# PH8411/image-matching

Measured on AMD Instinct MI355X. Metric: image-pairs/sec (640x480, 1024 kpts, 30 Sinkhorn iters), higher is better.
Workload: dtype f32

## Files before the change

### image-matching_amd/csrc/conv1ab_wino24h.hip

```cpp
#include "imx_kernels.h"
#include "wino24_pk.h"
#include <cstdio>
#include <cstdlib>
#include <type_traits>

namespace imx {

typedef float f32x4 __attribute__((ext_vector_type(4)));
typedef float f32x2 __attribute__((ext_vector_type(2)));
typedef _Float16 f16x8 __attribute__((ext_vector_type(8)));
typedef _Float16 f16x2 __attribute__((ext_vector_type(2)));
typedef unsigned u32x4v __attribute__((ext_vector_type(4)));

namespace {
constexpr int OH = 8, OW = 16;
constexpr int RH = OH + 2, RW = OW + 2;
constexpr int IMG_H = RH + 2, IMG_W = RW + 2;
constexpr int RSH = 34;
constexpr int RAWSZ = 192 * RSH;
constexpr int NPOS = 24;
constexpr int VPLANE = NPOS * 4 * 16 * 8;
constexpr int UPOS = 2 * 4 * 64 * 8;
constexpr int RING = 6;

// ... 8 lines not shown
  h[0] = (_Float16)x[0]; h[1] = (_Float16)x[1];
  const float r0 = __builtin_amdgcn_fdot2(h, lo, x[0], false);
  const float r1 = __builtin_amdgcn_fdot2(h, hi, x[1], false);
  m[0] = (_Float16)r0; m[1] = (_Float16)r1;
}
__device__ __forceinline__ float v_scale_of_bound(float bound) {
  unsigned e = (__builtin_bit_cast(unsigned, bound) >> 23) & 0xffu;
  e = e < 60u ? 60u : e > 200u ? 200u : e;
  return __builtin_bit_cast(float, (261u - e) << 23);
}

__global__ __launch_bounds__(256, 2) void conv1ab_wino24h(ConvArgs p, int tiles_x, int tiles_y, int ntiles) {
  extern __shared__ __attribute__((aligned(16))) unsigned char smem_1h[];
  _Float16* Vp = reinterpret_cast<_Float16*>(smem_1h);
  float* raw = reinterpret_cast<float*>(smem_1h + 2 * VPLANE * 2);
  float* img = raw + RAWSZ;
  float* wmax = img + IMG_H * IMG_W;

  const int tid = threadIdx.x, lane = tid & 63, wave = tid >> 6;
  const int cb = wave;
  const int H = p.H, W = p.W, Cout = p.Cout;
  const __amdgpu_buffer_rsrc_t ur = __builtin_amdgcn_make_buffer_rsrc((void*)p.wuh, 0, 2 * NPOS * UPOS * 2, 0x00020000);
  const int uoff_lane = (cb * 64 + lane) * 16;

  const int n = lane & 15, kq = lane >> 4;
  const float c2 = kq == 0 ? 1.f : 0.f, a2 = kq == 1 ? 1.f : 0.f;
  float wa[4][3];
  int toff[3];
#pragma unroll
  for (int ks = 0; ks < 3; ++ks) {
    const int tap = 4 * ks + kq;
    toff[ks] = tap < 9 ? (tap / 3) * IMG_W + tap % 3 : 0;
#pragma unroll
    for (int cbk = 0; cbk < 4; ++cbk) {
      const float* src = tap < 9 ? p.w1 + tap * 64 + cbk * 16 + n : p.b1 + cbk * 16 + n;
      const float v = *(tap <= 9 ? src : p.b1);
      wa[cbk][ks] = tap <= 9 ? v : 0.f;
    }
  }
  const int tk = lane & 3, tw = lane >> 2, twr = tw >> 2, twc = tw & 3;
  const int ra = wave == 0 ? 0 : wave == 2 ? 2 : 1, rb = wave == 0 ? 2 : wave == 1 ? 2 : wave == 2 ? 1 : 3;
  const float sg = wave == 1 ? 1.f : -1.f;
  const f32x2 sg2 = {sg, sg};
  const f32x2 m5 = {-5.f, -5.f};
  const float* rpa = raw + ((2 * twr + ra) * RW + 4 * twc) * RSH + 2 * tk;
  const float* rpb = raw + ((2 * twr + rb) * RW + 4 * twc) * RSH + 2 * tk;
  _Float16* vwr = Vp + (wave * 4 * 16 + tw) * 8 + 2 * tk;
  const _Float16* vrd = Vp + lane * 8;

  const int per = (ntiles + (int)gridDim.x - 1) / (int)gridDim.x;
  const int t_begin = (int)blockIdx.x * per, t_end = t_begin + per < ntiles ? t_begin + per : ntiles;
  int tx = t_begin % tiles_x, ty = (t_begin / tiles_x) % tiles_y, b = t_begin / (tiles_x * tiles_y);
  const int ipy = tid / IMG_W - 2, ipx = tid % IMG_W - 2;
  auto fetch_px = [&](int ftx, int fty, int fb, bool live) -> float {
// ... 24 lines not shown
  };
  const f32x4 bs4 = *reinterpret_cast<const f32x4*>(p.bias + cb * 16 + 4 * (lane >> 4));
  u32x4v ub[RING][2];
  auto u_load = [&](int slot, int chv, int pos) __attribute__((always_inline)) {
    const int so = __builtin_amdgcn_readfirstlane((chv * NPOS + pos) * (UPOS * 2));
    ub[slot][0] = __builtin_amdgcn_raw_buffer_load_b128(ur, uoff_lane, so, 0);
    ub[slot][1] = __builtin_amdgcn_raw_buffer_load_b128(ur, uoff_lane, so + 4 * 64 * 16, 0);
  };
#pragma unroll
  for (int g = 0; g < RING; ++g) u_load(g, 0, g);
  __builtin_amdgcn_s_waitcnt(0x0F70);

  f32x4 acc[NPOS];
  const f32x2 k8 = {8.f, 8.f};
  const f32x4 zero4c = {0.f, 0.f, 0.f, 0.f};
  float sv = 1.f;

  auto conv1a_half = [&](int half, int x0, int y0) __attribute__((always_inline)) {
    const f32x4 zero4 = {0.f, 0.f, 0.f, 0.f};
#pragma unroll
    for (int j = 0; j < 3; ++j) {
      const int pp = (3 * wave + j) * 16 + n;
      const int py = gpy[j], px = gpx[j];
      const int gy = y0 + py - 1, gx = x0 + px - 1;
      const float m = (pp < RH * RW && gy >= 0 && gy < H && gx >= 0 && gx < W) ? sv : 0.f;
      const float* ip = img + py * IMG_W + px;
      float bv[3];
      bv[0] = ip[toff[0]] * m;
      bv[1] = ip[toff[1]] * m;
      bv[2] = (ip[toff[2]] * c2 + a2) * m;
#pragma unroll
      for (int cl = 0; cl < 2; ++cl) {
        f32x4 d = zero4;
#pragma unroll
        for (int ks = 0; ks < 3; ++ks) d = __builtin_amdgcn_mfma_f32_16x16x4f32(half ? wa[2 + cl][ks] : wa[cl][ks], bv[ks], d, 0, 0, 0);
        typedef int i32x4 __attribute__((ext_vector_type(4)));
        d = __builtin_bit_cast(f32x4, __builtin_elementwise_max(__builtin_bit_cast(i32x4, d), (i32x4){0, 0, 0, 0}));
        float* o = raw + pp * RSH + cl * 16 + 4 * kq;
        *reinterpret_cast<f32x2*>(o) = (f32x2){d[0], d[1]};
        *reinterpret_cast<f32x2*>(o + 2) = (f32x2){d[2], d[3]};
      }
    }
  };
  auto transform = [&]() __attribute__((always_inline)) {
#pragma unroll
    for (int q = 0; q < 4; ++q) {
      f32x2 o[6], T[6];
#pragma unroll
      for (int bb = 0; bb < 6; ++bb)
        o[bb] = pk_fma(sg2, *reinterpret_cast<const f32x2*>(rpb + 8 * q + bb * RSH), *reinterpret_cast<const f32x2*>(rpa + 8 * q + bb * RSH));
      const W24Half hb = w24_batch_a(o, m5);
      w24_batch_b(o, hb, T);
#pragma unroll
      for (int jj = 0; jj < 6; ++jj) {
        f16x2 h, m;
        split_h2(T[jj], h, m);
        _Float16* d = vwr + ((jj * 4 * 4 + q) * 16) * 8;
// ... 18 lines not shown
      acc[pp + 1] = __builtin_amdgcn_mfma_f32_16x16x32_f16(ah1, bm[1], FIRST ? zero4c : acc[pp + 1], 0, 0, 0);
      acc[pp] = __builtin_amdgcn_mfma_f32_16x16x32_f16(am0, bh[0], acc[pp], 0, 0, 0);
      acc[pp + 1] = __builtin_amdgcn_mfma_f32_16x16x32_f16(am1, bh[1], acc[pp + 1], 0, 0, 0);
      acc[pp] = __builtin_amdgcn_mfma_f32_16x16x32_f16(ah0, bh[0], acc[pp], 0, 0, 0);
      acc[pp + 1] = __builtin_amdgcn_mfma_f32_16x16x32_f16(ah1, bh[1], acc[pp + 1], 0, 0, 0);
#pragma unroll
      for (int e = 0; e < 2; ++e) {
        const int np = pp + e + RING;
        if (np < NPOS) u_load((pp + e) % RING, c, np);
        else u_load((pp + e) % RING, c ^ 1, np - NPOS);
      }
      __builtin_amdgcn_sched_barrier(0);
    }
  };

  for (int t = t_begin; t < t_end; ++t) {
    const int x0 = tx * OW, y0 = ty * OH, bcur = b;
    if (tid < IMG_H * IMG_W) img[tid] = pre;
    {
      float mx = fabsf(pre);
#pragma unroll
      for (int o = 32; o >= 1; o >>= 1) mx = fmaxf(mx, __shfl_xor(mx, o));
      if (lane == 0) wmax[wave] = mx;
    }
    if (++tx == tiles_x) { tx = 0; if (++ty == tiles_y) { ty = 0; ++b; } }
    pre = fetch_px(tx, ty, b, t + 1 < t_end);
    __syncthreads();
    {
      const float imax = fmaxf(fmaxf(wmax[0], wmax[1]), fmaxf(wmax[2], wmax[3]));
      sv = __builtin_bit_cast(float, __builtin_amdgcn_readfirstlane(__builtin_bit_cast(int, v_scale_of_bound(fmaf(imax, p.c1a_l1, p.c1a_bmax)))));
    }
    conv1a_half(0, x0, y0);
    __syncthreads();
    transform();
    __syncthreads();
    mfma_phase(BoolC<true>{}, 0);
    conv1a_half(1, x0, y0);
    __syncthreads();
    transform();
    __syncthreads();
    mfma_phase(BoolC<false>{}, 1);

    {
      const float inv = p.u_scale_inv / sv;
      const f32x4 inv4 = {inv, inv, inv, inv};
      f32x4 y[2][4];
      w24_output_transform(acc, k8, y);
      const f32x4 zero4 = {0.f, 0.f, 0.f, 0.f};
      const int wr = (lane & 15) >> 2, wc = lane & 3;
      const int Ho = H >> 1, Wo = W >> 1;
      const __amdgpu_buffer_rsrc_t ors = __builtin_amdgcn_make_buffer_rsrc((void*)(p.out + (size_t)bcur * Ho * Wo * Cout), 0, Ho * Wo * Cout * 4, 0x00020000);
      const bool outb = p.out_blocked != 0;
// ... 8 lines not shown
        const int ox = (x0 >> 1) + 2 * wc + hh;
        const unsigned off = (oy < Ho && ox < Wo) ? (unsigned)((oy * Wo + ox) * opx + choff) : 0x7ffffff0u;
        __builtin_amdgcn_raw_buffer_store_b128(__builtin_bit_cast(u32x4, v), ors, (int)off, 0, 0);
        if (p.amax_out) {
          if (bcur != am_b) { am_flush(); am_b = bcur; }
          am_run = max(am_run, __builtin_bit_cast(unsigned, fmaxf(fmaxf(v[0], v[1]), fmaxf(v[2], v[3]))));
        }
      }
    }
  }
  if (p.amax_out) am_flush();
}
}

bool conv1ab_wino24h_supported(const ConvArgs& a) {
  return a.first && a.pool && a.Cin == 64 && a.Cout == 64 && a.wuh && a.u_scale_inv > 0.f && a.c1a_l1 > 0.f;
}

hipError_t launch_conv1ab_wino24h(const ConvArgs& a, hipStream_t s) {
  if (!conv1ab_wino24h_supported(a)) return hipErrorInvalidValue;
  const int tiles_x = (a.W + OW - 1) / OW, tiles_y = (a.H + OH - 1) / OH, ntiles = tiles_x * tiles_y * a.B;
  const size_t lds = (size_t)2 * VPLANE * 2 + (size_t)(RAWSZ + IMG_H * IMG_W + 4) * sizeof(float);
  static int ncu = 0;
  if (!ncu) {
    int dev = 0;
    hipDeviceProp_t prop;
    if (hipGetDevice(&dev) != hipSuccess || hipGetDeviceProperties(&prop, dev) != hipSuccess) return hipErrorUnknown;
    ncu = prop.multiProcessorCount;
  }
  static unsigned long long attr = 0;
  raise_lds_limit(reinterpret_cast<const void*>(conv1ab_wino24h), (int)lds, attr);
  const dim3 grid((unsigned)(ntiles < 2 * ncu ? ntiles : 2 * ncu));
  last_form = "conv1ab_wino24h:f16x2";
  hipLaunchKernelGGL(conv1ab_wino24h, grid, dim3(256), lds, s, a, tiles_x, tiles_y, ntiles);
  return hipGetLastError();
}

// ... 2 lines not shown
```

### image-matching_amd/csrc/conv1ab_wino24p.hip

```cpp
#include "imx_kernels.h"
#include "wino24_pk.h"
#include <cstdint>
#include <cstdio>
#include <cstdlib>
#include <type_traits>

namespace imx {

typedef float f32x4 __attribute__((ext_vector_type(4)));
typedef float f32x2 __attribute__((ext_vector_type(2)));
typedef _Float16 f16x8 __attribute__((ext_vector_type(8)));
typedef _Float16 f16x2 __attribute__((ext_vector_type(2)));
typedef unsigned u32x4v __attribute__((ext_vector_type(4)));

namespace {
constexpr int OH = 8, OW = 16;
constexpr int RH = OH + 2, RW = OW + 2;
constexpr int IMG_H = RH + 2, IMG_W = RW + 2;
constexpr int IMG_N = IMG_H * IMG_W;
constexpr int RSH = 34;
constexpr int RAWSZ = 192 * RSH;
constexpr int NPOS = 24, NLP = 12, NG = 2;
constexpr int VPLANE = NPOS * 4 * 16 * 8;
constexpr int VGRP = 2 * VPLANE;
// ... 17 lines not shown
}
__device__ __forceinline__ int lane_now() {
  int l;
  asm volatile("v_mbcnt_lo_u32_b32 %0, -1, 0\n\tv_mbcnt_hi_u32_b32 %0, -1, %0" : "=v"(l));
  return l;
}
__device__ __forceinline__ float v_scale_of_bound(float bound) {
  unsigned e = (__builtin_bit_cast(unsigned, bound) >> 23) & 0xffu;
  e = e < 60u ? 60u : e > 200u ? 200u : e;
  return __builtin_bit_cast(float, (261u - e) << 23);
}

__global__ __launch_bounds__(512) void conv1ab_wino24p(ConvArgs p, int tiles_x, int tiles_y, int ntiles) {
  extern __shared__ __attribute__((aligned(16))) unsigned char smem_1p[];
  float* raw = reinterpret_cast<float*>(smem_1p + NG * VGRP * 2);
  float* img = raw + NG * RAWSZ;
  float* wmax = img + NG * IMG_N;
  unsigned* amax_tab = reinterpret_cast<unsigned*>(wmax + 8);
  const unsigned lds0 = (unsigned)(uintptr_t)(__attribute__((address_space(3))) unsigned char*)smem_1p;

  const int tid = threadIdx.x, lane = tid & 63;
  const int wave_s = __builtin_amdgcn_readfirstlane(tid >> 6);
  const int cb = wave_s & 3, ph = wave_s >> 2;
  const int tq = wave_s & 3, tg = wave_s >> 2;
  const int H = p.H, W = p.W, Cout = p.Cout;
  const __amdgpu_buffer_rsrc_t ur = __builtin_amdgcn_make_buffer_rsrc((void*)p.wuh, 0, 2 * NPOS * UPOS * 2, 0x00020000);
  const int uoff_lane = (cb * 64 + lane) * 16 + ph * NLP * (UPOS * 2);
  typedef const float __attribute__((address_space(4)))* cf32p;
  const cf32p bias_c = (cf32p)(uintptr_t)p.bias;

  const int n = lane & 15, kq = lane >> 4;
  const float c2 = kq == 0 ? 1.f : 0.f, a2 = kq == 1 ? 1.f : 0.f;
  float wa[4][3];
  int toff[3];
#pragma unroll
  for (int ks = 0; ks < 3; ++ks) {
    const int tap = 4 * ks + kq;
    toff[ks] = tap < 9 ? (tap / 3) * IMG_W + tap % 3 : 0;
#pragma unroll
    for (int cbk = 0; cbk < 4; ++cbk) {
      const float* src = tap < 9 ? p.w1 + tap * 64 + cbk * 16 + n : p.b1 + cbk * 16 + n;
      const float v = *(tap <= 9 ? src : p.b1);
      wa[cbk][ks] = tap <= 9 ? v : 0.f;
    }
  }
  const int tk = lane & 3, tw = lane >> 2, twr = tw >> 2, twc = tw & 3;
  const f32x2 m5 = {-5.f, -5.f}, one2 = {1.f, 1.f}, mone2 = {-1.f, -1.f};
  const float* rp = raw + tg * RAWSZ + ((2 * twr) * RW + 4 * twc) * RSH + 8 * tq + 2 * tk;
  _Float16* const vwr = (_Float16*)((__attribute__((address_space(3))) unsigned char*)(uintptr_t)(lds0 + (unsigned)(tg * (VGRP * 2) + tq * 256 + lane * 4)));
  const _Float16 *vrdK, *vrdS;
  {
    unsigned a = lds0 + (unsigned)(ph * (VGRP * 2) + ph * NLP * 1024 + lane * 16);
    unsigned b = lds0 + (unsigned)((1 - ph) * (VGRP * 2) + ph * NLP * 1024 + lane * 16);
    asm volatile("" : "+v"(a), "+v"(b));
    vrdK = (const _Float16*)((__attribute__((address_space(3))) unsigned char*)(uintptr_t)a);
    vrdS = (const _Float16*)((__attribute__((address_space(3))) unsigned char*)(uintptr_t)b);
  }

  const int npairs = (ntiles + NG - 1) / NG;
  const int per = (npairs + (int)gridDim.x - 1) / (int)gridDim.x;
// ... 34 lines not shown
  }
  u32x4v ub[RING][2];
  auto u_load = [&](int slot, int chv, int lp) __attribute__((always_inline)) {
    const int pos = lp;
    const int so = __builtin_amdgcn_readfirstlane((chv * NPOS + pos) * (UPOS * 2));
    ub[slot][0] = __builtin_amdgcn_raw_buffer_load_b128(ur, uoff_lane, so, 0);
    ub[slot][1] = __builtin_amdgcn_raw_buffer_load_b128(ur, uoff_lane, so + 4 * 64 * 16, 0);
  };
  for (int i = tid; i < AMAX_SLOTS; i += 512) amax_tab[i] = 0;
#pragma unroll
  for (int g = 0; g < RING; ++g) u_load(g, 0, g);

  f32x4 accK[NLP], accS[NLP];
  const f32x2 k8 = {8.f, 8.f};
  const f32x4 zero4c = {0.f, 0.f, 0.f, 0.f};
  float sv = 1.f;
  float* const rawt = raw + tg * RAWSZ;
  const float* const imgt = img + tg * IMG_N;

  auto conv1a_block = [&](int half, int j, int x0, int y0, float svb) __attribute__((always_inline)) {
    const f32x4 zero4 = {0.f, 0.f, 0.f, 0.f};
    {
      const int pp = (3 * tq + j) * 16 + n;
      const int py = gpy[j], px = gpx[j];
      const int gy = y0 + py - 1, gx = x0 + px - 1;
      const float m = (pp < RH * RW && gy >= 0 && gy < H && gx >= 0 && gx < W) ? svb : 0.f;
      const float* ip = imgt + py * IMG_W + px;
      float bv[3];
      bv[0] = ip[toff[0]] * m;
      bv[1] = ip[toff[1]] * m;
      bv[2] = (ip[toff[2]] * c2 + a2) * m;
#pragma unroll
      for (int cl = 0; cl < 2; ++cl) {
        f32x4 d = zero4;
#pragma unroll
        for (int ks = 0; ks < 3; ++ks) d = __builtin_amdgcn_mfma_f32_16x16x4f32(half ? wa[2 + cl][ks] : wa[cl][ks], bv[ks], d, 0, 0, 0);
        typedef int i32x4 __attribute__((ext_vector_type(4)));
        d = __builtin_bit_cast(f32x4, __builtin_elementwise_max(__builtin_bit_cast(i32x4, d), (i32x4){0, 0, 0, 0}));
        float* o = rawt + pp * RSH + cl * 16 + 4 * kq;
        *reinterpret_cast<f32x2*>(o) = (f32x2){d[0], d[1]};
        *reinterpret_cast<f32x2*>(o + 2) = (f32x2){d[2], d[3]};
      }
    }
  };
  auto conv1a_half = [&](int half, int x0, int y0, float svb) __attribute__((always_inline)) {
#pragma unroll
    for (int j = 0; j < 3; ++j) conv1a_block(half, j, x0, y0, svb);
  };
  auto v_store2 = [&](int pos, f16x2 h, f16x2 m) __attribute__((always_inline)) {
    *reinterpret_cast<f16x2*>(vwr + pos * 512) = h;
    *reinterpret_cast<f16x2*>(vwr + VPLANE + pos * 512) = m;
  };
  auto transform = [&]() __attribute__((always_inline)) {
    f32x2 r1[6], r2[6], rx[6];
    auto row_load = [&](f32x2 (&d)[6], int row) __attribute__((always_inline)) {
#pragma unroll
      for (int bb = 0; bb < 6; ++bb) d[bb] = *reinterpret_cast<const f32x2*>(rp + (row * RW + bb) * RSH);
    };
    auto row_out = [&](int i, f32x2 sg2, const f32x2 (&bq)[6], const f32x2 (&aq)[6]) __attribute__((always_inline)) {
      f32x2 o[6], T[6];
// ... 5 lines not shown
      for (int jj = 0; jj < 6; ++jj) {
        f16x2 h, m;
        split_h2(T[jj], h, m);
        v_store2(jj * 4 + i, h, m);
      }
    };
    row_load(r1, 1);
    row_load(r2, 2);
    row_load(rx, 0);
    row_out(1, one2, r2, r1);
    row_out(2, mone2, r1, r2);
    row_out(0, mone2, r2, rx);
    row_load(rx, 3);
    row_out(3, mone2, rx, r1);
  };
  auto mfma_phase = [&](auto firstc, int c, int x0, int y0, float svb) __attribute__((always_inline)) {
    constexpr bool FIRST = decltype(firstc)::value;
    f16x8 bq[2][4];
    auto b_load = [&](int buf, int lp) __attribute__((always_inline)) {
      const int po = lp * 512;
      bq[buf][0] = *reinterpret_cast<const f16x8*>(vrdK + po);
      bq[buf][1] = *reinterpret_cast<const f16x8*>(vrdK + VPLANE + po);
      bq[buf][2] = *reinterpret_cast<const f16x8*>(vrdS + po);
      bq[buf][3] = *reinterpret_cast<const f16x8*>(vrdS + VPLANE + po);
    };
    b_load(0, 0);
#pragma unroll
    for (int lp = 0; lp < NLP; ++lp) {
      const int buf = lp & 1;
      if (lp + 1 < NLP) b_load(buf ^ 1, lp + 1);
      __builtin_amdgcn_sched_barrier(0);
// ... 11 lines not shown
        else u_load(lp % RING, c ^ 1, np - NLP);
      }
      __builtin_amdgcn_sched_barrier(0);
      if ((lp & 3) == 1) {
        conv1a_block(FIRST ? 1 : 0, lp >> 2, x0, y0, svb);
        __builtin_amdgcn_sched_barrier(0);
      }
    }
  };

  unsigned amax_run = 0;
  const int Ho = H >> 1, Wo = W >> 1;
  const bool outb = p.out_blocked != 0;
  const int opx = outb ? 32 : Cout * 4;
  __syncthreads();
  auto image_to_lds = [&]() __attribute__((always_inline)) {
    const int ln = lane_now(), t8n = (wave_s & 3) * 64 + ln;
    if (t8n < IMG_N) img[tg * IMG_N + t8n] = pre;
    unsigned mb = __builtin_bit_cast(unsigned, fabsf(pre));
    mb = max(mb, (unsigned)__builtin_amdgcn_update_dpp(0, (int)mb, 0xb1, 0xf, 0xf, true));
    mb = max(mb, (unsigned)__builtin_amdgcn_update_dpp(0, (int)mb, 0x4e, 0xf, 0xf, true));
    mb = max(mb, (unsigned)__builtin_amdgcn_update_dpp(0, (int)mb, 0x141, 0xf, 0xf, true));
    mb = max(mb, (unsigned)__builtin_amdgcn_update_dpp(0, (int)mb, 0x140, 0xf, 0xf, true));
    const unsigned m01 = max((unsigned)__builtin_amdgcn_readlane((int)mb, 0), (unsigned)__builtin_amdgcn_readlane((int)mb, 16));
    const unsigned m23 = max((unsigned)__builtin_amdgcn_readlane((int)mb, 32), (unsigned)__builtin_amdgcn_readlane((int)mb, 48));
    if (ln == 0) wmax[wave_s] = __builtin_bit_cast(float, max(m01, m23));
  };
  auto scale_from_lds = [&]() __attribute__((always_inline)) -> float {
    const float* wm = wmax + 4 * tg;
    const float imax = fmaxf(fmaxf(wm[0], wm[1]), fmaxf(wm[2], wm[3]));
    return __builtin_bit_cast(float, __builtin_amdgcn_readfirstlane(__builtin_bit_cast(int, v_scale_of_bound(fmaf(imax, p.c1a_l1, p.c1a_bmax)))));
  };
  int x0 = tx * OW, y0 = ty * OH, bcur = tlive ? b : 0, lcur = tlive;
  image_to_lds();
  next_tile();
  pre = fetch_px(q_begin + 1 < q_end);
  __syncthreads();
  sv = scale_from_lds();
  conv1a_half(0, x0, y0, sv);
  __syncthreads();
  for (int q = q_begin; q < q_end; ++q) {
    transform();
    __syncthreads();
    mfma_phase(BoolC<true>{}, 0, x0, y0, sv);
    __syncthreads();
    const int x0n = tx * OW, y0n = ty * OH, bn = tlive ? b : 0, ln = tlive;
    image_to_lds();
    next_tile();
    pre = fetch_px(q + 2 < q_end);
    transform();
    __syncthreads();
    const float svn = scale_from_lds();
    mfma_phase(BoolC<false>{}, 1, x0n, y0n, svn);
    __syncthreads();

    typedef __attribute__((address_space(3))) f32x4* lds4p;
    const int lq = lane_now();
    const unsigned xw = lds0 + (unsigned)(wave_s * XCH + lq * 16), xr = lds0 + (unsigned)((wave_s ^ 4) * XCH + lq * 16);
    f32x4 bs4;
    {
      const int bo = __builtin_amdgcn_readfirstlane(cb * 16);
      typedef const f32x4 __attribute__((address_space(4)))* cf4p;
      const cf4p b4 = (cf4p)(bias_c + bo);
      const f32x4 b0 = b4[0], b1 = b4[1], b2 = b4[2], b3 = b4[3];
      const int kq2 = lq >> 4;
#pragma unroll
      for (int qq = 0; qq < 4; ++qq) bs4[qq] = kq2 == 0 ? b0[qq] : kq2 == 1 ? b1[qq] : kq2 == 2 ? b2[qq] : b3[qq];
// ... 17 lines not shown
      gs0[jj] = *(lds4p)(uintptr_t)(xr + (2 * jj) * 1024);
      gs1[jj] = *(lds4p)(uintptr_t)(xr + (2 * jj + 1) * 1024);
    }
    __syncthreads();

    f32x4 y[2][4];
    {
      auto cols = [&](const f32x4 (&a0)[3], const f32x4 (&a1)[3], const f32x4 (&b0)[3], const f32x4 (&b1)[3]) __attribute__((always_inline)) {
        const f32x4 s0[6] = {a0[0], a0[1], a0[2], b0[0], b0[1], b0[2]}, s1[6] = {a1[0], a1[1], a1[2], b1[0], b1[1], b1[2]};
        w24_out_cols(s0, s1, k8, y);
      };
      if (ph == 0) { cols(sK0, sK1, gs0, gs1); asm volatile("" ::: "memory"); }
      else { cols(gs0, gs1, sK0, sK1); asm volatile("; order 1" ::: "memory"); }
    }
    {
      const float inv = p.u_scale_inv / sv;
      const f32x4 inv4 = {inv, inv, inv, inv};
      const f32x4 zero4 = {0.f, 0.f, 0.f, 0.f};
      const int wr = (lq & 15) >> 2, wc = lq & 3;
      const int bu = __builtin_amdgcn_readfirstlane(bcur), lv = __builtin_amdgcn_readfirstlane(lcur);
      const __amdgpu_buffer_rsrc_t ors = __builtin_amdgcn_make_buffer_rsrc((void*)(p.out + (size_t)bu * Ho * Wo * Cout), 0, lv ? Ho * Wo * Cout * 4 : 0, 0x00020000);
      const int choff = outb ? (cb * 2 + (lq >> 5)) * (Ho * Wo * 32) + ((lq >> 4) & 1) * 16 : (cb * 16 + 4 * (lq >> 4)) * 4;
      typedef unsigned u32x4 __attribute__((__vector_size__(4 * sizeof(unsigned))));
      const int oy = (y0 >> 1) + wr;
#pragma unroll
      for (int hh = 0; hh < 2; ++hh) {
        const f32x4 mx4 = __builtin_elementwise_max(__builtin_elementwise_max(y[0][2 * hh], y[0][2 * hh + 1]), __builtin_elementwise_max(y[1][2 * hh], y[1][2 * hh + 1]));
        const f32x4 v = __builtin_elementwise_max(__builtin_elementwise_fma(mx4, inv4, bs4), zero4);
        const int ox = (x0 >> 1) + 2 * wc + hh;
        const unsigned off = (oy < Ho && ox < Wo) ? (unsigned)((oy * Wo + ox) * opx + choff) : 0x7ffffff0u;
        __builtin_amdgcn_raw_buffer_store_b128(__builtin_bit_cast(u32x4, v), ors, (int)off, 0, 0);
        amax_run = max(amax_run, __builtin_bit_cast(unsigned, fmaxf(fmaxf(v[0], v[1]), fmaxf(v[2], v[3]))));
      }
      if (p.amax_out) {
        unsigned mb = amax_run;
        mb = max(mb, (unsigned)__builtin_amdgcn_update_dpp(0, (int)mb, 0xb1, 0xf, 0xf, true));
        mb = max(mb, (unsigned)__builtin_amdgcn_update_dpp(0, (int)mb, 0x4e, 0xf, 0xf, true));
        mb = max(mb, (unsigned)__builtin_amdgcn_update_dpp(0, (int)mb, 0x141, 0xf, 0xf, true));
        mb = max(mb, (unsigned)__builtin_amdgcn_update_dpp(0, (int)mb, 0x140, 0xf, 0xf, true));
        const unsigned m01 = max((unsigned)__builtin_amdgcn_readlane((int)mb, 0), (unsigned)__builtin_amdgcn_readlane((int)mb, 16));
        const unsigned m23 = max((unsigned)__builtin_amdgcn_readlane((int)mb, 32), (unsigned)__builtin_amdgcn_readlane((int)mb, 48));
        const unsigned mw = max(m01, m23);
        if (lv && mw && lq == 0) atomicMax(amax_tab + (bu & (AMAX_SLOTS - 1)), mw);
        amax_run = 0;
      }
    }
    x0 = x0n; y0 = y0n; bcur = bn; lcur = ln; sv = svn;
  }
  if (p.amax_out) {
    __syncthreads();
    for (int i = tid; i < AMAX_SLOTS; i += 512)
      if (amax_tab[i]) atomicMax(p.amax_out + i, amax_tab[i]);
  }
}
}

bool conv1ab_wino24p_supported(const ConvArgs& a) { return conv1ab_wino24h_supported(a); }

bool conv1ab_wino24p_preferred(const ConvArgs& a) {
  if (!conv1ab_wino24p_supported(a)) return false;
  static int ncu = 0;
  if (!ncu) {
    int dev = 0;
    hipDeviceProp_t prop;
    if (hipGetDevice(&dev) != hipSuccess || hipGetDeviceProperties(&prop, dev) != hipSuccess) return false;
    ncu = prop.multiProcessorCount;
  }
  const long long tiles = (long long)((a.W + OW - 1) / OW) * ((a.H + OH - 1) / OH) * a.B;
  return (tiles + NG - 1) / NG >= 2LL * ncu;
}

hipError_t launch_conv1ab_wino24p(const ConvArgs& a, hipStream_t s) {
  if (!conv1ab_wino24p_supported(a)) return hipErrorInvalidValue;
  const int tiles_x = (a.W + OW - 1) / OW, tiles_y = (a.H + OH - 1) / OH, ntiles = tiles_x * tiles_y * a.B;
  const int npairs = (ntiles + NG - 1) / NG;
  const size_t lds = (size_t)NG * VGRP * 2 + (size_t)(NG * RAWSZ + NG * IMG_N + 8) * sizeof(float) + AMAX_SLOTS * sizeof(unsigned);
  static int ncu = 0;
  if (!ncu) {
    int dev = 0;
    hipDeviceProp_t prop;
    if (hipGetDevice(&dev) != hipSuccess || hipGetDeviceProperties(&prop, dev) != hipSuccess) return hipErrorUnknown;
    ncu = prop.multiProcessorCount;
  }
  static unsigned long long attr = 0;
  raise_lds_limit(reinterpret_cast<const void*>(conv1ab_wino24p), (int)lds, attr);
  const dim3 grid((unsigned)(npairs < ncu ? npairs : ncu));
  last_form = "conv1ab_wino24p:f16x2";
  hipLaunchKernelGGL(conv1ab_wino24p, grid, dim3(512), lds, s, a, tiles_x, tiles_y, ntiles);
  return hipGetLastError();
}

// ... 2 lines not shown
```

### image-matching_amd/csrc/imx_api.cpp

```cpp
#include "../../include/imx.h"
#include "imx_kernels.h"
#include "gnn_tail_pack.h"
#include "wino24_pack.h"

#include <hip/hip_runtime.h>
#include <dlfcn.h>

#include <cctype>
#include <cmath>
#include <cstdarg>
#include <cstdio>
#include <cstdlib>
#include <cstring>
#include <exception>
#include <map>
#include <memory>
#include <new>
#include <atomic>
#include <string>
#include <vector>

using namespace imx;

namespace imx {
// ... 60 lines not shown

}

struct imx_handle_s {
  int device = 0;
  imx_config_t cfg{};
  std::string err;
  std::map<std::string, std::vector<int64_t>> expected[2];
  std::map<std::string, HostTensor> raw[2];
  bool finalized[2] = {false, false};
  std::vector<void*> weight_allocs[2];
  int upload_net = 0;
  float *w1 = nullptr, *b1 = nullptr;
  struct { const float* smap = nullptr; float* nms = nullptr; void* scratch = nullptr; int B = 0, H = 0, W = 0, radius = 0; bool pending = false; } nms_lazy;
  float c1a_l1 = 0.f, c1a_bmax = 0.f, c1a_spread = 1.f;
  ConvW conv[8];
  GemmW pb, db;
  float *kenc0_w = nullptr, *kenc0_b = nullptr;
  int kenc_c1 = 0;
  std::vector<GemmW> kenc;
  std::vector<GnnLayer> layers;
  GemmW final_proj;
  float bin_score = 1.f;
  std::map<std::string, DevBuf> bufs;
  int det_B = 0, det_H = 0, det_W = 0, det_Hc = 0, det_Wc = 0, det_Ksel = 0;
  Options opt;
  std::string opt_text;
  bool debug = false, timing = false;
  int poison = -1;
  std::map<std::string, Tap> taps;
// ... 343 lines not shown
      float l1 = 0.f;
      for (int t = 0; t < 9; ++t) l1 += std::fabs(w[t * 64 + c]);
      h->c1a_l1 = std::max(h->c1a_l1, l1);
      h->c1a_bmax = std::max(h->c1a_bmax, std::fabs(b[c]));
    }
    h->c1a_l1 = std::max(h->c1a_l1, 1e-30f);
    std::vector<double> comax(64, 0.0);
    double wmax = 0.0;
    for (int t = 0; t < 9; ++t)
      for (int c = 0; c < 64; ++c) {
        comax[c] = std::max(comax[c], (double)std::fabs(w[t * 64 + c]));
        wmax = std::max(wmax, comax[c]);
      }
    std::nth_element(comax.begin(), comax.begin() + 32, comax.end());
    h->c1a_spread = comax[32] > 0 ? (float)std::min(3.0e38, wmax / comax[32]) : (wmax > 0 ? 3.0e38f : 1.f);
  }
  const int cin[8] = {1, 64, 64, 64, 64, 128, 128, 128}, cout[8] = {64, 64, 64, 64, 128, 128, 128, 128};
  for (int i = 1; i < 8; ++i)
    if (make_conv(h, h->conv[i - 1], raw, ck[i], bk[i], cin[i], cout[i])) return -1;
  {
    std::vector<float> w((size_t)9 * 128 * 512), b(512);
    put_conv3(raw, "convPa", bn ? "bnPa" : "", 128, 256, 512, 0, w, b);
    put_conv3(raw, "convDa", bn ? "bnDa" : "", 128, 256, 512, 256, w, b);
    h->conv[7].w = upload(h, w);
    h->conv[7].wu24 = upload(h, wino24_transform(w, 128, 512));
    h->conv[7].wuh = upload_u16(h, wino24h_pack(w, 128, 512, &h->conv[7].su_inv, &h->conv[7].u_spread));
    h->conv[7].b = upload(h, b);
    h->conv[7].cin = 128;
    h->conv[7].cout = 512;
    if (!h->conv[7].w || !h->conv[7].wu24 || !h->conv[7].b) return fail(h, "weight upload failed (heads)");
// ... 255 lines not shown
    const int li = layer++;
    for (int sl = 0; sl < (amax ? nslice : 1); ++sl) {
    ConvArgs a{};
    const int b0 = amax ? sl * kSlice : 0, nb = amax ? std::min(kSlice, B - b0) : B;
    const bool in_z = !first && swz_pair(li - 1, hh, ww, nb), out_z = !first && !pool && !last && swz_pair(li, hh, ww, nb);
    const size_t ztile = (size_t)((hh + 7) / 8) * ((ww + 15) / 16) * 2048;
    const bool in_cand = li == 2 || li == 4 || li == 6, out_cand = li == 1 || li == 3 || li == 5;
    const size_t in_img = in_cand ? ztile * (w.cin / 16) : (size_t)hh * ww * (first ? 1 : w.cin);
    const size_t out_img = out_cand ? ztile * (w.cout / 16) : (size_t)(pool ? hh / 2 : hh) * (pool ? ww / 2 : ww) * w.cout;
    if (amax) {
      unsigned* am = amax + (size_t)sl * 8 * 256;
      a.amax_out = last ? nullptr : am + (size_t)li * 256;
      a.amax_in = li > 0 ? am + (size_t)(li - 1) * 256 : nullptr;
      a.wuh = w.wuh; a.u_scale_inv = w.su_inv;
      a.c1a_l1 = h->c1a_l1; a.c1a_bmax = h->c1a_bmax;
    }
    a.in_blocked = in_z ? 2 : (blocked && !first) ? 1 : 0;
    a.out_blocked = out_z ? 2 : (blocked && !last) ? 1 : 0;
    if (first) {
      if (b0 >= split) { a.in = img1 + (size_t)(b0 - split) * in_img; a.in2 = nullptr; a.split = nb; }
      else { a.in = in + (size_t)b0 * in_img; a.in2 = img1; a.split = split - b0; }
    } else {
      a.in = in + (size_t)b0 * in_img; a.in2 = nullptr; a.split = 0;
    }
    a.w = w.w; a.wu24 = w.wu24; a.bias = w.b; a.w1 = h->w1; a.b1 = h->b1; a.out = out + (size_t)b0 * out_img;
    a.B = nb; a.H = hh; a.W = ww; a.Cin = w.cin; a.Cout = w.cout; a.relu = 1; a.pool = pool ? 1 : 0; a.first = first ? 1 : 0;
    const bool fused1 = a.first && a.pool && !h->opt.conv_direct;
    const bool wino = !a.first && !h->opt.conv_direct && conv3x3_wino24_supported(a);
    const bool winoh = wino && amax && conv3x3_wino24h_supported(a);
    if (amax && !fused1 && !winoh) return fail(h, "%s: the fp16-plane Winograd chain needs every layer to take part (internal)", name);
// ... 995 lines not shown
```

### image-matching_amd/csrc/imx_kernels.h

```cpp
#pragma once
#include <hip/hip_runtime.h>
#include <stdint.h>

namespace imx {

struct Options {
  int mfma_f32 = 0;
  int latency_forms = -1;
  int gnn_tail = -1;
  int attention = -1;
  int conv_direct = 0;
  int conv_f16 = 1;
  int conv_swizzle = 1;
  int qkv_amax = 0;
  int sinkhorn_group = 0;
  int sinkhorn_prefetch = -1;
  int sinkhorn_merge = -1;
  int keypoints = -1;
  int attention_qblocks = -1;
  int ha_masks = 0;
  int linear = -1;
};

extern thread_local const char* last_form;
// ... 13 lines not shown
  int split;
  const float* w;
  const float* wu24;
  const float* bias;
  const float* w1;
  const float* b1;
  float* out;
  int B, H, W, Cin, Cout;
  int relu, pool, first;
  int in_blocked, out_blocked;
  const void* wuh;
  float u_scale_inv;
  const unsigned* amax_in;
  unsigned* amax_out;
  float c1a_l1, c1a_bmax;
};
hipError_t launch_conv3x3(const ConvArgs& a, hipStream_t s);
hipError_t launch_conv1ab_wino24(const ConvArgs& a, hipStream_t s);
bool conv1ab_wino24h_supported(const ConvArgs& a);
hipError_t launch_conv1ab_wino24h(const ConvArgs& a, hipStream_t s);
bool conv1ab_wino24p_supported(const ConvArgs& a);
bool conv1ab_wino24p_preferred(const ConvArgs& a);
hipError_t launch_conv1ab_wino24p(const ConvArgs& a, hipStream_t s);
bool conv3x3_wino24_supported(const ConvArgs& a);
hipError_t launch_conv3x3_wino24(const ConvArgs& a, hipStream_t s);
bool conv3x3_wino24h_supported(const ConvArgs& a);
hipError_t launch_conv3x3_wino24h(const ConvArgs& a, hipStream_t s);
bool conv3x3_wino24p_supported(const ConvArgs& a);
bool conv3x3_wino24p_preferred(const ConvArgs& a);
hipError_t launch_conv3x3_wino24p(const ConvArgs& a, hipStream_t s);
// ... 227 lines not shown
```

Before: 2666.

## Compute conv1a with split-fp16 MFMA instead of f32 MFMA

Replaces the fp32 16x16x4 MFMA first-layer convolution with 16x16x32 fp16 MFMAs. The input patch is stored in LDS as hi/mid/lo fp16 splits, and the weights are pre-packed on the host as three-way fp16 splits with a power-of-two scale. The goal is to cut the MFMA count and register-held weights for conv1a while staying close to fp32 accuracy. The per-patch max is now computed before the store, which moves the wmax reduction and adds a sync. This adds LDS for the split patch and, in the p variant, for the weights, and it risks small accuracy loss.

```diff
diff --git a/image-matching_amd/csrc/conv1a_f16.h b/image-matching_amd/csrc/conv1a_f16.h
--- /dev/null
+++ b/image-matching_amd/csrc/conv1a_f16.h
@@ -0,0 +1,76 @@
+#pragma once
+#include <hip/hip_runtime.h>
+
+namespace imx {
+namespace c1a {
+
+typedef float f32x4 __attribute__((ext_vector_type(4)));
+typedef _Float16 f16x8 __attribute__((ext_vector_type(8)));
+typedef _Float16 f16x2 __attribute__((ext_vector_type(2)));
+typedef unsigned u32x4 __attribute__((ext_vector_type(4)));
+
+constexpr int PW = 20, PN = 12 * PW;
+constexpr int PATCH_WORDS = 2 * PN;
+constexpr int A_BYTES = 4 * 2 * 64 * 16;
+
+__device__ __forceinline__ unsigned in_exp(float imax) {
+  const unsigned e = (__builtin_bit_cast(unsigned, imax) >> 23) & 0xffu;
+  return e < 125u ? 125u : e > 154u ? 154u : e;
+}
+__device__ __forceinline__ float in_scale(unsigned e) { return __builtin_bit_cast(float, (267u - e) << 23); }
+__device__ __forceinline__ float in_scale_inv(unsigned e) { return __builtin_bit_cast(float, (e - 13u) << 23); }
+__device__ __forceinline__ unsigned in_scale_pk(unsigned e) {
+  const unsigned c = (155u - e) << 10;
+  return c | (c << 16);
+}
+
+__device__ __forceinline__ void patch_store(unsigned* patch, int i, float v, float imax) {
+  const float xs = fminf(fmaxf(v * in_scale(in_exp(imax)), -65504.f), 65504.f);
+  const _Float16 h = (_Float16)xs;
+  const float r = xs - (float)h;
+  const _Float16 m = (_Float16)r, l = (_Float16)(r - (float)m);
+  if (i < PN) {
+    patch[i] = __builtin_bit_cast(unsigned, (f16x2){h, m});
+    patch[PN + i] = __builtin_bit_cast(unsigned, (f16x2){l, h});
+  }
+}
+
+__device__ __forceinline__ void lane_offsets(int kq, int (&off)[8]) {
+#pragma unroll
+  for (int r = 0; r < 8; ++r) {
+    const int R = 16 * (r >> 2) + 4 * kq + (r & 3);
+    const int t = R < 9 ? R : R < 18 ? R - 9 : R < 27 ? R - 18 : 0;
+    off[r] = (R >= 18 && R < 27 ? PN : 0) + (t / 3) * PW + t % 3;
+  }
+}
+
+__device__ __forceinline__ void block(const unsigned* patch, const unsigned char* a_frag, float* raw_px, int half, int lane, int pix,
+                                      const int (&off)[8], unsigned spk, float mult) {
+  const int kq = lane >> 4;
+  u32x4 b0, b1;
+#pragma unroll
+  for (int r = 0; r < 4; ++r) {
+    b0[r] = patch[pix + off[r]];
+    b1[r] = patch[pix + off[4 + r]];
+  }
+  b1[3] = kq == 2 ? spk : b1[3];
+  b1[0] = kq == 3 ? spk : b1[0];
+  const f16x8 bf0 = __builtin_bit_cast(f16x8, b0), bf1 = __builtin_bit_cast(f16x8, b1);
+  const f32x4 zero4 = {0.f, 0.f, 0.f, 0.f}, m4 = {mult, mult, mult, mult};
+#pragma unroll
+  for (int cl = 0; cl < 2; ++cl) {
+    const unsigned char* ap = a_frag + (((2 * half + cl) * 2) * 64 + lane) * 16;
+    const f16x8 a0 = *reinterpret_cast<const f16x8*>(ap), a1 = *reinterpret_cast<const f16x8*>(ap + 64 * 16);
+    f32x4 d = __builtin_amdgcn_mfma_f32_16x16x32_f16(a0, bf0, zero4, 0, 0, 0);
+    d = __builtin_amdgcn_mfma_f32_16x16x32_f16(a1, bf1, d, 0, 0, 0) * m4;
+    typedef int i32x4 __attribute__((ext_vector_type(4)));
+    d = __builtin_bit_cast(f32x4, __builtin_elementwise_max(__builtin_bit_cast(i32x4, d), (i32x4){0, 0, 0, 0}));
+    float* o = raw_px + cl * 16 + 4 * kq;
+    typedef float f32x2 __attribute__((ext_vector_type(2)));
+    *reinterpret_cast<f32x2*>(o) = (f32x2){d[0], d[1]};
+    *reinterpret_cast<f32x2*>(o + 2) = (f32x2){d[2], d[3]};
+  }
+}
+
+}
+}
diff --git a/image-matching_amd/csrc/conv1a_pack.h b/image-matching_amd/csrc/conv1a_pack.h
--- /dev/null
+++ b/image-matching_amd/csrc/conv1a_pack.h
@@ -0,0 +1,53 @@
+#pragma once
+#include "gnn_tail_pack.h"
+
+namespace imx {
+
+inline std::vector<uint16_t> c1a_pack_f16(const float* w, const float* b, float* s_inv, float* spread) {
+  std::vector<double> comax(64, 0.0), bab(64, 0.0);
+  double mx = 0.0;
+  for (int c = 0; c < 64; ++c) {
+    for (int t = 0; t < 9; ++t) comax[c] = std::max(comax[c], (double)std::fabs(w[t * 64 + c]));
+    bab[c] = std::fabs((double)b[c]);
+    mx = std::max(mx, std::max(comax[c], bab[c]));
+  }
+  std::nth_element(comax.begin(), comax.begin() + 32, comax.end());
+  std::nth_element(bab.begin(), bab.begin() + 32, bab.end());
+  double typ = comax[32];
+  if (*std::max_element(bab.begin(), bab.end()) > 0) typ = std::min(typ, bab[32]);
+  int e = 0;
+  if (mx > 0) std::frexp(mx, &e);
+  const bool finite = std::isfinite(mx) && e >= -40 && e <= 40;
+  *spread = !finite ? 3.0e38f : typ > 0 ? (float)std::min(3.0e38, mx / typ) : (mx > 0 ? 3.0e38f : 1.f);
+  const double sc = finite ? std::ldexp(1.0, 14 - e) : 1.0;
+  *s_inv = (float)(1.0 / sc);
+  std::vector<uint16_t> pk((size_t)4 * 2 * 64 * 8, 0);
+  auto split = [sc](float v, uint16_t (&pl)[3]) {
+    float x = (float)((double)v * sc);
+    for (int q = 0; q < 3; ++q) {
+      pl[q] = gt_f16_rne(x);
+      x -= gt_f16_f(pl[q]);
+    }
+  };
+  for (int c = 0; c < 64; ++c) {
+    uint16_t wp[9][3], bp[3];
+    for (int t = 0; t < 9; ++t) split(w[t * 64 + c], wp[t]);
+    split(b[c], bp);
+    uint16_t slot[64];
+    for (int R = 0; R < 32; ++R) {
+      uint16_t lo = 0, hi = 0;
+      if (R < 9) { lo = wp[R][0]; hi = wp[R][0]; }
+      else if (R < 18) { lo = wp[R - 9][1]; hi = wp[R - 9][1]; }
+      else if (R < 27) { lo = wp[R - 18][0]; hi = wp[R - 18][2]; }
+      else if (R == 27) { lo = bp[0]; hi = bp[1]; }
+      else if (R == 28) { lo = bp[2]; }
+      slot[2 * R] = lo;
+      slot[2 * R + 1] = hi;
+    }
+    const int cb = c >> 4, n = c & 15;
+    for (int k = 0; k < 64; ++k) pk[((((size_t)cb * 2 + (k >> 5)) * 64) + ((k >> 3) & 3) * 16 + n) * 8 + (k & 7)] = slot[k];
+  }
+  return pk;
+}
+
+}
diff --git a/image-matching_amd/csrc/conv1ab_wino24h.hip b/image-matching_amd/csrc/conv1ab_wino24h.hip
--- a/image-matching_amd/csrc/conv1ab_wino24h.hip
+++ b/image-matching_amd/csrc/conv1ab_wino24h.hip
@@ -1,5 +1,6 @@
 #include "imx_kernels.h"
 #include "wino24_pk.h"
+#include "conv1a_f16.h"
 #include <cstdio>
 #include <cstdlib>
 #include <type_traits>
@@ -46,8 +47,9 @@
   extern __shared__ __attribute__((aligned(16))) unsigned char smem_1h[];
   _Float16* Vp = reinterpret_cast<_Float16*>(smem_1h);
   float* raw = reinterpret_cast<float*>(smem_1h + 2 * VPLANE * 2);
-  float* img = raw + RAWSZ;
-  float* wmax = img + IMG_H * IMG_W;
+  unsigned* img = reinterpret_cast<unsigned*>(raw + RAWSZ);
+  float* wmax = reinterpret_cast<float*>(img + c1a::PATCH_WORDS);
+  const unsigned char* const c1a_w = reinterpret_cast<const unsigned char*>(p.w1h);
 
   const int tid = threadIdx.x, lane = tid & 63, wave = tid >> 6;
   const int cb = wave;
@@ -55,21 +57,7 @@
   const __amdgpu_buffer_rsrc_t ur = __builtin_amdgcn_make_buffer_rsrc((void*)p.wuh, 0, 2 * NPOS * UPOS * 2, 0x00020000);
   const int uoff_lane = (cb * 64 + lane) * 16;
 
-  const int n = lane & 15, kq = lane >> 4;
-  const float c2 = kq == 0 ? 1.f : 0.f, a2 = kq == 1 ? 1.f : 0.f;
-  float wa[4][3];
-  int toff[3];
-#pragma unroll
-  for (int ks = 0; ks < 3; ++ks) {
-    const int tap = 4 * ks + kq;
-    toff[ks] = tap < 9 ? (tap / 3) * IMG_W + tap % 3 : 0;
-#pragma unroll
-    for (int cbk = 0; cbk < 4; ++cbk) {
-      const float* src = tap < 9 ? p.w1 + tap * 64 + cbk * 16 + n : p.b1 + cbk * 16 + n;
-      const float v = *(tap <= 9 ? src : p.b1);
-      wa[cbk][ks] = tap <= 9 ? v : 0.f;
-    }
-  }
+  const int n = lane & 15;
   const int tk = lane & 3, tw = lane >> 2, twr = tw >> 2, twc = tw & 3;
   const int ra = wave == 0 ? 0 : wave == 2 ? 2 : 1, rb = wave == 0 ? 2 : wave == 1 ? 2 : wave == 2 ? 1 : 3;
   const float sg = wave == 1 ? 1.f : -1.f;
@@ -124,33 +112,28 @@
   f32x4 acc[NPOS];
   const f32x2 k8 = {8.f, 8.f};
   const f32x4 zero4c = {0.f, 0.f, 0.f, 0.f};
-  float sv = 1.f;
+  float sv = 1.f, cm = 1.f;
+  unsigned spk = 0;
 
   auto conv1a_half = [&](int half, int x0, int y0) __attribute__((always_inline)) {
-    const f32x4 zero4 = {0.f, 0.f, 0.f, 0.f};
 #pragma unroll
     for (int j = 0; j < 3; ++j) {
       const int pp = (3 * wave + j) * 16 + n;
       const int py = gpy[j], px = gpx[j];
       const int gy = y0 + py - 1, gx = x0 + px - 1;
-      const float m = (pp < RH * RW && gy >= 0 && gy < H && gx >= 0 && gx < W) ? sv : 0.f;
-      const float* ip = img + py * IMG_W + px;
-      float bv[3];
-      bv[0] = ip[toff[0]] * m;
-      bv[1] = ip[toff[1]] * m;
-      bv[2] = (ip[toff[2]] * c2 + a2) * m;
-#pragma unroll
-      for (int cl = 0; cl < 2; ++cl) {
-        f32x4 d = zero4;
-#pragma unroll
-        for (int ks = 0; ks < 3; ++ks) d = __builtin_amdgcn_mfma_f32_16x16x4f32(half ? wa[2 + cl][ks] : wa[cl][ks], bv[ks], d, 0, 0, 0);
-        typedef int i32x4 __attribute__((ext_vector_type(4)));
-        d = __builtin_bit_cast(f32x4, __builtin_elementwise_max(__builtin_bit_cast(i32x4, d), (i32x4){0, 0, 0, 0}));
-        float* o = raw + pp * RSH + cl * 16 + 4 * kq;
-        *reinterpret_cast<f32x2*>(o) = (f32x2){d[0], d[1]};
-        *reinterpret_cast<f32x2*>(o + 2) = (f32x2){d[2], d[3]};
-      }
-    }
+      const float m = (pp < RH * RW && gy >= 0 && gy < H && gx >= 0 && gx < W) ? cm : 0.f;
+      int la = lane;
+      asm volatile("" : "+v"(la));
+      int coff[8];
+      c1a::lane_offsets(la >> 4, coff);
+      c1a::block(img, c1a_w, raw + pp * RSH, half, la, py * IMG_W + px, coff, spk, m);
+    }
+  };
+  auto patch_max_to_lds = [&]() __attribute__((always_inline)) {
+    float mx = fabsf(pre);
+#pragma unroll
+    for (int o = 32; o >= 1; o >>= 1) mx = fmaxf(mx, __shfl_xor(mx, o));
+    if (lane == 0) wmax[wave] = mx;
   };
   auto transform = [&]() __attribute__((always_inline)) {
 #pragma unroll
@@ -199,21 +182,20 @@
     }
   };
 
+  patch_max_to_lds();
+  __syncthreads();
   for (int t = t_begin; t < t_end; ++t) {
     const int x0 = tx * OW, y0 = ty * OH, bcur = b;
-    if (tid < IMG_H * IMG_W) img[tid] = pre;
-    {
-      float mx = fabsf(pre);
-#pragma unroll
-      for (int o = 32; o >= 1; o >>= 1) mx = fmaxf(mx, __shfl_xor(mx, o));
-      if (lane == 0) wmax[wave] = mx;
-    }
+    const float imax = fmaxf(fmaxf(wmax[0], wmax[1]), fmaxf(wmax[2], wmax[3]));
+    c1a::patch_store(img, tid, pre, imax);
     if (++tx == tiles_x) { tx = 0; if (++ty == tiles_y) { ty = 0; ++b; } }
     pre = fetch_px(tx, ty, b, t + 1 < t_end);
     __syncthreads();
     {
-      const float imax = fmaxf(fmaxf(wmax[0], wmax[1]), fmaxf(wmax[2], wmax[3]));
       sv = __builtin_bit_cast(float, __builtin_amdgcn_readfirstlane(__builtin_bit_cast(int, v_scale_of_bound(fmaf(imax, p.c1a_l1, p.c1a_bmax)))));
+      const unsigned e = (unsigned)__builtin_amdgcn_readfirstlane((int)c1a::in_exp(imax));
+      cm = sv * c1a::in_scale_inv(e) * p.c1a_sinv;
+      spk = c1a::in_scale_pk(e);
     }
     conv1a_half(0, x0, y0);
     __syncthreads();
@@ -221,6 +203,7 @@
     __syncthreads();
     mfma_phase(BoolC<true>{}, 0);
     conv1a_half(1, x0, y0);
+    patch_max_to_lds();
     __syncthreads();
     transform();
     __syncthreads();
@@ -259,13 +242,13 @@
 }
 
 bool conv1ab_wino24h_supported(const ConvArgs& a) {
-  return a.first && a.pool && a.Cin == 64 && a.Cout == 64 && a.wuh && a.u_scale_inv > 0.f && a.c1a_l1 > 0.f;
+  return a.first && a.pool && a.Cin == 64 && a.Cout == 64 && a.wuh && a.u_scale_inv > 0.f && a.c1a_l1 > 0.f && a.w1h && a.c1a_sinv > 0.f;
 }
 
 hipError_t launch_conv1ab_wino24h(const ConvArgs& a, hipStream_t s) {
   if (!conv1ab_wino24h_supported(a)) return hipErrorInvalidValue;
   const int tiles_x = (a.W + OW - 1) / OW, tiles_y = (a.H + OH - 1) / OH, ntiles = tiles_x * tiles_y * a.B;
-  const size_t lds = (size_t)2 * VPLANE * 2 + (size_t)(RAWSZ + IMG_H * IMG_W + 4) * sizeof(float);
+  const size_t lds = (size_t)2 * VPLANE * 2 + (size_t)(RAWSZ + c1a::PATCH_WORDS + 4) * sizeof(float);
   static int ncu = 0;
   if (!ncu) {
     int dev = 0;
diff --git a/image-matching_amd/csrc/conv1ab_wino24p.hip b/image-matching_amd/csrc/conv1ab_wino24p.hip
--- a/image-matching_amd/csrc/conv1ab_wino24p.hip
+++ b/image-matching_amd/csrc/conv1ab_wino24p.hip
@@ -1,5 +1,6 @@
 #include "imx_kernels.h"
 #include "wino24_pk.h"
+#include "conv1a_f16.h"
 #include <cstdint>
 #include <cstdio>
 #include <cstdlib>
@@ -55,9 +56,10 @@
 __global__ __launch_bounds__(512) void conv1ab_wino24p(ConvArgs p, int tiles_x, int tiles_y, int ntiles) {
   extern __shared__ __attribute__((aligned(16))) unsigned char smem_1p[];
   float* raw = reinterpret_cast<float*>(smem_1p + NG * VGRP * 2);
-  float* img = raw + NG * RAWSZ;
-  float* wmax = img + NG * IMG_N;
+  unsigned* img = reinterpret_cast<unsigned*>(raw + NG * RAWSZ);
+  float* wmax = reinterpret_cast<float*>(img + NG * c1a::PATCH_WORDS);
   unsigned* amax_tab = reinterpret_cast<unsigned*>(wmax + 8);
+  const unsigned char* const c1a_w = reinterpret_cast<const unsigned char*>(amax_tab + AMAX_SLOTS);
   const unsigned lds0 = (unsigned)(uintptr_t)(__attribute__((address_space(3))) unsigned char*)smem_1p;
 
   const int tid = threadIdx.x, lane = tid & 63;
@@ -71,20 +73,9 @@
   const cf32p bias_c = (cf32p)(uintptr_t)p.bias;
 
   const int n = lane & 15, kq = lane >> 4;
-  const float c2 = kq == 0 ? 1.f : 0.f, a2 = kq == 1 ? 1.f : 0.f;
-  float wa[4][3];
-  int toff[3];
-#pragma unroll
-  for (int ks = 0; ks < 3; ++ks) {
-    const int tap = 4 * ks + kq;
-    toff[ks] = tap < 9 ? (tap / 3) * IMG_W + tap % 3 : 0;
-#pragma unroll
-    for (int cbk = 0; cbk < 4; ++cbk) {
-      const float* src = tap < 9 ? p.w1 + tap * 64 + cbk * 16 + n : p.b1 + cbk * 16 + n;
-      const float v = *(tap <= 9 ? src : p.b1);
-      wa[cbk][ks] = tap <= 9 ? v : 0.f;
-    }
-  }
+  int coff[8];
+  c1a::lane_offsets(kq, coff);
+  if (tid < c1a::A_BYTES / 16) reinterpret_cast<u32x4v*>(const_cast<unsigned char*>(c1a_w))[tid] = reinterpret_cast<const u32x4v*>(p.w1h)[tid];
   const int tk = lane & 3, tw = lane >> 2, twr = tw >> 2, twc = tw & 3;
   const f32x2 m5 = {-5.f, -5.f}, one2 = {1.f, 1.f}, mone2 = {-1.f, -1.f};
   const float* rp = raw + tg * RAWSZ + ((2 * twr) * RW + 4 * twc) * RSH + 8 * tq + 2 * tk;
@@ -149,36 +140,19 @@
   f32x4 accK[NLP], accS[NLP];
   const f32x2 k8 = {8.f, 8.f};
   const f32x4 zero4c = {0.f, 0.f, 0.f, 0.f};
-  float sv = 1.f;
+  struct C1aScale { float sv, cm; unsigned spk; };
+  C1aScale sc = {1.f, 1.f, 0u};
   float* const rawt = raw + tg * RAWSZ;
-  const float* const imgt = img + tg * IMG_N;
-
-  auto conv1a_block = [&](int half, int j, int x0, int y0, float svb) __attribute__((always_inline)) {
-    const f32x4 zero4 = {0.f, 0.f, 0.f, 0.f};
-    {
-      const int pp = (3 * tq + j) * 16 + n;
-      const int py = gpy[j], px = gpx[j];
-      const int gy = y0 + py - 1, gx = x0 + px - 1;
-      const float m = (pp < RH * RW && gy >= 0 && gy < H && gx >= 0 && gx < W) ? svb : 0.f;
-      const float* ip = imgt + py * IMG_W + px;
-      float bv[3];
-      bv[0] = ip[toff[0]] * m;
-      bv[1] = ip[toff[1]] * m;
-      bv[2] = (ip[toff[2]] * c2 + a2) * m;
-#pragma unroll
-      for (int cl = 0; cl < 2; ++cl) {
-        f32x4 d = zero4;
-#pragma unroll
-        for (int ks = 0; ks < 3; ++ks) d = __builtin_amdgcn_mfma_f32_16x16x4f32(half ? wa[2 + cl][ks] : wa[cl][ks], bv[ks], d, 0, 0, 0);
-        typedef int i32x4 __attribute__((ext_vector_type(4)));
-        d = __builtin_bit_cast(f32x4, __builtin_elementwise_max(__builtin_bit_cast(i32x4, d), (i32x4){0, 0, 0, 0}));
-        float* o = rawt + pp * RSH + cl * 16 + 4 * kq;
-        *reinterpret_cast<f32x2*>(o) = (f32x2){d[0], d[1]};
-        *reinterpret_cast<f32x2*>(o + 2) = (f32x2){d[2], d[3]};
-      }
-    }
-  };
-  auto conv1a_half = [&](int half, int x0, int y0, float svb) __attribute__((always_inline)) {
+  unsigned* const imgt = img + tg * c1a::PATCH_WORDS;
+
+  auto conv1a_block = [&](int half, int j, int x0, int y0, const C1aScale& sb) __attribute__((always_inline)) {
+    const int pp = (3 * tq + j) * 16 + n;
+    const int py = gpy[j], px = gpx[j];
+    const int gy = y0 + py - 1, gx = x0 + px - 1;
+    const float m = (pp < RH * RW && gy >= 0 && gy < H && gx >= 0 && gx < W) ? sb.cm : 0.f;
+    c1a::block(imgt, c1a_w, rawt + pp * RSH, half, lane, py * IMG_W + px, coff, sb.spk, m);
+  };
+  auto conv1a_half = [&](int half, int x0, int y0, const C1aScale& svb) __attribute__((always_inline)) {
 #pragma unroll
     for (int j = 0; j < 3; ++j) conv1a_block(half, j, x0, y0, svb);
   };
@@ -214,7 +188,7 @@
     row_load(rx, 3);
     row_out(3, mone2, rx, r1);
   };
-  auto mfma_phase = [&](auto firstc, int c, int x0, int y0, float svb) __attribute__((always_inline)) {
+  auto mfma_phase = [&](auto firstc, int c, int x0, int y0, const C1aScale& svb) __attribute__((always_inline)) {
     constexpr bool FIRST = decltype(firstc)::value;
     f16x8 bq[2][4];
     auto b_load = [&](int buf, int lp) __attribute__((always_inline)) {
@@ -256,9 +230,8 @@
   const bool outb = p.out_blocked != 0;
   const int opx = outb ? 32 : Cout * 4;
   __syncthreads();
-  auto image_to_lds = [&]() __attribute__((always_inline)) {
-    const int ln = lane_now(), t8n = (wave_s & 3) * 64 + ln;
-    if (t8n < IMG_N) img[tg * IMG_N + t8n] = pre;
+  auto patch_max_to_lds = [&]() __attribute__((always_inline)) {
+    const int ln = lane_now();
     unsigned mb = __builtin_bit_cast(unsigned, fabsf(pre));
     mb = max(mb, (unsigned)__builtin_amdgcn_update_dpp(0, (int)mb, 0xb1, 0xf, 0xf, true));
     mb = max(mb, (unsigned)__builtin_amdgcn_update_dpp(0, (int)mb, 0x4e, 0xf, 0xf, true));
@@ -268,23 +241,35 @@
     const unsigned m23 = max((unsigned)__builtin_amdgcn_readlane((int)mb, 32), (unsigned)__builtin_amdgcn_readlane((int)mb, 48));
     if (ln == 0) wmax[wave_s] = __builtin_bit_cast(float, max(m01, m23));
   };
-  auto scale_from_lds = [&]() __attribute__((always_inline)) -> float {
+  auto patch_max = [&]() __attribute__((always_inline)) -> float {
     const float* wm = wmax + 4 * tg;
-    const float imax = fmaxf(fmaxf(wm[0], wm[1]), fmaxf(wm[2], wm[3]));
-    return __builtin_bit_cast(float, __builtin_amdgcn_readfirstlane(__builtin_bit_cast(int, v_scale_of_bound(fmaf(imax, p.c1a_l1, p.c1a_bmax)))));
+    return fmaxf(fmaxf(wm[0], wm[1]), fmaxf(wm[2], wm[3]));
+  };
+  auto image_to_lds = [&]() __attribute__((always_inline)) {
+    const int t8n = (wave_s & 3) * 64 + lane_now();
+    c1a::patch_store(img + tg * c1a::PATCH_WORDS, t8n, pre, patch_max());
+  };
+  auto scale_from_lds = [&]() __attribute__((always_inline)) -> C1aScale {
+    const float imax = patch_max();
+    const float svv = __builtin_bit_cast(float, __builtin_amdgcn_readfirstlane(__builtin_bit_cast(int, v_scale_of_bound(fmaf(imax, p.c1a_l1, p.c1a_bmax)))));
+    const unsigned e = (unsigned)__builtin_amdgcn_readfirstlane((int)c1a::in_exp(imax));
+    return {svv, svv * c1a::in_scale_inv(e) * p.c1a_sinv, c1a::in_scale_pk(e)};
   };
   int x0 = tx * OW, y0 = ty * OH, bcur = tlive ? b : 0, lcur = tlive;
+  patch_max_to_lds();
+  __syncthreads();
   image_to_lds();
   next_tile();
   pre = fetch_px(q_begin + 1 < q_end);
   __syncthreads();
-  sv = scale_from_lds();
-  conv1a_half(0, x0, y0, sv);
+  sc = scale_from_lds();
+  conv1a_half(0, x0, y0, sc);
   __syncthreads();
   for (int q = q_begin; q < q_end; ++q) {
     transform();
     __syncthreads();
-    mfma_phase(BoolC<true>{}, 0, x0, y0, sv);
+    mfma_phase(BoolC<true>{}, 0, x0, y0, sc);
+    patch_max_to_lds();
     __syncthreads();
     const int x0n = tx * OW, y0n = ty * OH, bn = tlive ? b : 0, ln = tlive;
     image_to_lds();
@@ -292,7 +277,7 @@
     pre = fetch_px(q + 2 < q_end);
     transform();
     __syncthreads();
-    const float svn = scale_from_lds();
+    const C1aScale svn = scale_from_lds();
     mfma_phase(BoolC<false>{}, 1, x0n, y0n, svn);
     __syncthreads();
 
@@ -340,7 +325,7 @@
       else { cols(gs0, gs1, sK0, sK1); asm volatile("; order 1" ::: "memory"); }
     }
     {
-      const float inv = p.u_scale_inv / sv;
+      const float inv = p.u_scale_inv / sc.sv;
       const f32x4 inv4 = {inv, inv, inv, inv};
       const f32x4 zero4 = {0.f, 0.f, 0.f, 0.f};
       const int wr = (lq & 15) >> 2, wc = lq & 3;
@@ -371,7 +356,7 @@
         amax_run = 0;
       }
     }
-    x0 = x0n; y0 = y0n; bcur = bn; lcur = ln; sv = svn;
+    x0 = x0n; y0 = y0n; bcur = bn; lcur = ln; sc = svn;
   }
   if (p.amax_out) {
     __syncthreads();
@@ -400,7 +385,7 @@
   if (!conv1ab_wino24p_supported(a)) return hipErrorInvalidValue;
   const int tiles_x = (a.W + OW - 1) / OW, tiles_y = (a.H + OH - 1) / OH, ntiles = tiles_x * tiles_y * a.B;
   const int npairs = (ntiles + NG - 1) / NG;
-  const size_t lds = (size_t)NG * VGRP * 2 + (size_t)(NG * RAWSZ + NG * IMG_N + 8) * sizeof(float) + AMAX_SLOTS * sizeof(unsigned);
+  const size_t lds = (size_t)NG * VGRP * 2 + (size_t)(NG * RAWSZ + NG * c1a::PATCH_WORDS + 8) * sizeof(float) + AMAX_SLOTS * sizeof(unsigned) + c1a::A_BYTES;
   static int ncu = 0;
   if (!ncu) {
     int dev = 0;
diff --git a/image-matching_amd/csrc/imx_api.cpp b/image-matching_amd/csrc/imx_api.cpp
--- a/image-matching_amd/csrc/imx_api.cpp
+++ b/image-matching_amd/csrc/imx_api.cpp
@@ -2,6 +2,7 @@
 #include "imx_kernels.h"
 #include "gnn_tail_pack.h"
 #include "wino24_pack.h"
+#include "conv1a_pack.h"
 
 #include <hip/hip_runtime.h>
 #include <dlfcn.h>
@@ -98,6 +99,8 @@
   float *w1 = nullptr, *b1 = nullptr;
   struct { const float* smap = nullptr; float* nms = nullptr; void* scratch = nullptr; int B = 0, H = 0, W = 0, radius = 0; bool pending = false; } nms_lazy;
   float c1a_l1 = 0.f, c1a_bmax = 0.f, c1a_spread = 1.f;
+  void* w1h = nullptr;
+  float c1a_sinv = 0.f;
   ConvW conv[8];
   GemmW pb, db;
   float *kenc0_w = nullptr, *kenc0_b = nullptr;
@@ -471,6 +474,10 @@
       }
     std::nth_element(comax.begin(), comax.begin() + 32, comax.end());
     h->c1a_spread = comax[32] > 0 ? (float)std::min(3.0e38, wmax / comax[32]) : (wmax > 0 ? 3.0e38f : 1.f);
+    float pk_spread = 1.f;
+    h->w1h = upload_u16(h, c1a_pack_f16(w.data(), b.data(), &h->c1a_sinv, &pk_spread));
+    if (!h->w1h) return fail(h, "weight upload failed (conv1a planes)");
+    h->c1a_spread = std::max(h->c1a_spread, pk_spread);
   }
   const int cin[8] = {1, 64, 64, 64, 64, 128, 128, 128}, cout[8] = {64, 64, 64, 64, 128, 128, 128, 128};
   for (int i = 1; i < 8; ++i)
@@ -756,6 +763,7 @@
       a.amax_in = li > 0 ? am + (size_t)(li - 1) * 256 : nullptr;
       a.wuh = w.wuh; a.u_scale_inv = w.su_inv;
       a.c1a_l1 = h->c1a_l1; a.c1a_bmax = h->c1a_bmax;
+      a.w1h = h->w1h; a.c1a_sinv = h->c1a_sinv;
     }
     a.in_blocked = in_z ? 2 : (blocked && !first) ? 1 : 0;
     a.out_blocked = out_z ? 2 : (blocked && !last) ? 1 : 0;
diff --git a/image-matching_amd/csrc/imx_kernels.h b/image-matching_amd/csrc/imx_kernels.h
--- a/image-matching_amd/csrc/imx_kernels.h
+++ b/image-matching_amd/csrc/imx_kernels.h
@@ -51,6 +51,8 @@
   const unsigned* amax_in;
   unsigned* amax_out;
   float c1a_l1, c1a_bmax;
+  const void* w1h;
+  float c1a_sinv;
 };
 hipError_t launch_conv3x3(const ConvArgs& a, hipStream_t s);
 hipError_t launch_conv1ab_wino24(const ConvArgs& a, hipStream_t s);
```

Result: slower. 2629 (-1.4%).
